# cbg-ethz/metMHN

Hardware: AMD Instinct MI355X
Metric: full-cohort log-lik+grad evals/sec at n=20 events; kronvec HBM GB/s (higher is better)
Workload: dtype f64

## Files before the change

metmhn_amd/csrc/engine.hip:

```cpp
#include <algorithm>
#include <chrono>
#include <cmath>
#include <cstdio>
#include <cstdlib>
#include <cstring>
#include <string>
#include <vector>

#include "../../include/metmhn_amd.h"
#include "host.h"
#include "comm.h"
#include "plan.h"
#include "sampler.h"
#include "rowmix.h"

namespace mmhn {

static thread_local std::string g_err;

struct CListDev {
  DevArr<CItem> items;
  DevArr<int> deps;
};
struct StagedDev {
  DevArr<int> pats, paired, probs;
  DevArr<int2> map, lmap, grc;
  CListDev cl[2];
};
struct BatchDev {
  DevArr<PatRec> pats;
  DevArr<Desc> dJ, dS;
  DevArr<int2> mapJ, mapS, lmapJ, mapX, grcJ, lmapT;
  DevArr<int> sp_list[3][SP_NCLASS], paired, olist, ptoff;
  DevArr<uint32_t> ptiles;
  DevArr<WDesc> wd;
  DevArr<WChain> wchains;
  DevArr<int4> pcl;
  DevArr<double> wrow;
  CListDev clJ[2];
  StagedDev stg[2];
};

struct Config {
  PlanCfg plan;
  bool zero_copy = true;
  bool poison = false;
  bool force_timing = false;
  bool coop_fault = false;
  int coop_wgs = 0;
  bool coop = true;
  long long sim_chunk = 1ll << 26;
  int stream_blocks = 256 * 8;
  bool trace_host = false;
  Config() {
    plan.use_jacobi = env_is("MMHN_SOLVER", "jacobi");
    plan.psolve_min = (int)env_int("MMHN_PSOLVE_MIN", plan.psolve_min);
    plan.wsolve_min = (int)env_int("MMHN_WSOLVE_MIN", env_set("MMHN_PSOLVE_MIN") ? plan.psolve_min : plan.wsolve_min);
    plan.wsolve_mode = (int)env_int("MMHN_WSOLVE", plan.wsolve_mode);
    plan.wsolve_wgs = (int)env_int("MMHN_WSOLVE_WGS", plan.wsolve_wgs);
    plan.prep_split_max = (int)env_int("MMHN_PREP_SPLIT", plan.prep_split_max);
    plan.pcl_per = std::max(1, (int)env_int("MMHN_PCL_PER", plan.pcl_per));
    plan.small_path = env_flag("MMHN_SMALL", plan.small_path);
    zero_copy = env_flag("MMHN_ZEROCOPY", zero_copy);
    poison = env_flag("MMHN_POISON", poison);
    force_timing = env_flag("MMHN_TIME_KERNELS", force_timing);
    coop_fault = env_flag("MMHN_COOP_FAULT", coop_fault);
    coop_wgs = (int)env_int("MMHN_COOP_WGS", coop_wgs);
    coop = env_flag("MMHN_COOP", coop);
    sim_chunk = std::max(1ll, env_int("MMHN_SIM_CHUNK", sim_chunk));
    stream_blocks = (int)env_int("MMHN_STREAM_BLOCKS", stream_blocks);
    trace_host = env_set("MMHN_TRACE_HOST");
  }
};

struct EngineBase {
  virtual ~EngineBase() = default;
  int dtype = 0;
  int device = 0;
  hipStream_t stream = nullptr;
  Config cfg;
};

template <typename T> struct Engine;
template <typename T> void clear_row_groups(Engine<T>& E);
template <typename T> void launch_mix(Engine<T>& E, const Lane& L);

template <typename T>
struct PList {
  const Desc* d; const int2* map; int ntiles; int maxk; long long vec;
  const int2* lmap; const std::vector<int>* lof; const T* tab;
  const CList* cl = nullptr;
  const CListDev* dcl = nullptr;
  int kslot = MMHN_K_OTHER_SOLVE;
};

template <typename... K>
static void raise_lds(size_t bytes, K... kernels) {
  for (const void* k : {reinterpret_cast<const void*>(kernels)...})
    HIPCHECK(hipFuncSetAttribute(k, hipFuncAttributeMaxDynamicSharedMemorySize, (int)bytes));
}

template <typename T>
struct Engine : EngineBase {
  using PList = mmhn::PList<T>;
  int n = 0, N = 0;
  DevArr<Params<T>> d_par;
  Params<T>* h_par = nullptr;
  void* h_par_dev = nullptr;
  DevArr<uint16_t> d_perm;
  DevArr<int> d_lvl;
  std::vector<int8_t> dat;
  long long n_pat = 0;
  int n_cols = 0;
  struct Counts { double em = 0, pat = 0, unknown = 0; } plain, weighted, grouped;
  std::vector<Batch> batches;
  std::vector<BatchDev> dev;
  DevArr<T> pi, lidgJ, qJ, rhsJ, rhsS, pS, lidgS, qS, seedS, GS, dots, bmJ, bmS, tabJ, tabS;
  DevArr<T> piM, qM;
  DevArr<T> zarena;
  struct View { T* p = nullptr; } GJ, DJ, Abuf;
  int pi_owner = -1, qJ_owner = -1;
  DevArr<double> lp, out, sums, abi_sums, redbuf;
  DevArr<double> resp;
  long long n_unknown = 0;
  std::vector<double> row_w;
  std::vector<long long> grp_ptr;
  std::vector<int> grp_rows;
  std::vector<double> grp_w;
  struct GroupsDev {
    DevArr<long long> gptr, mptr;
    DevArr<int> grows, mgrp;
    DevArr<double> gw, lpc, lpg, omega, lambda, rho;
  } gd;
  bool want_rho = false;
  DevArr<JLink<T>> links;
  double* h_abi = nullptr;
  double* h_abi_dev = nullptr;
  Lane main, side[3];
  DevArr<CoopCtl> coop_ctl;
  DevArr<unsigned> coop_flags[2];
  unsigned coop_epoch = 0;
  int coop_slot = 0;
  unsigned* h_abort = nullptr;
  unsigned* h_abort_dev = nullptr;
  bool coop_used = false;
  bool coop_alone = false;
  bool sums_pending = false;
  std::chrono::steady_clock::time_point sums_t0, sums_issued;
  int sums_len = 0;
  int pack_mode = 0;
  double pack_a = 0, pack_b = 0;
  double* pack_dst = nullptr;
  bool packed_in_eval = false;
  double reduce_flag = 0.0, reduce_flag_sum = 0.0;
  bool flag_pending = false;
  ncclComm_t comm = nullptr;
  int comm_rank = 0, comm_size = 1;
  bool time_kernels = true;
  mmhn_counters cnt{};
  std::vector<std::pair<hipEvent_t, hipEvent_t>> ev_pool;
  size_t ev_used = 0;
  std::vector<double> ev_bytes;
  std::vector<int> ev_slot;

  static long long zarena_elems(long long nJ, long long asize, int N) { return up4(3 * nJ * N * N) + up4(3 * nJ * N) + up4(asize); }
  static long long zclear_elems(const Batch& b, int N) { return zarena_elems((long long)b.dJ.size(), b.aclr, N); }

  Engine(int dev_id, int n_mut) : n(n_mut), N(n_mut + 1) {
    device = dev_id;
    cnt.comm_rank = -1;
    REQUIRE(n_mut >= 1 && n_mut < MAXN, "n_mut must be in [1, 31]");
    DevGuard guard(device);
    HIPCHECK(hipStreamCreateWithFlags(&stream, hipStreamNonBlocking));
    main.s = stream;
    main.flags = 0;
    d_par.alloc(NPSET);
    HIPCHECK(hipHostMalloc(reinterpret_cast<void**>(&h_par), NPSET * sizeof(Params<T>), hipHostMallocDefault));
    HIPCHECK(hipHostGetDevicePointer(&h_par_dev, h_par, 0));
    static_assert(sizeof(Params<T>) % sizeof(uint4) == 0, "parameter block: whole 16-byte words");
    sums.alloc(2 * stride());
    size_t free_b = 0, total_b = 0;
    HIPCHECK(hipMemGetInfo(&free_b, &total_b));
    cfg.plan.ws_limit = (size_t)(0.7 * (double)free_b);
    hipDeviceProp_t prop;
    HIPCHECK(hipGetDeviceProperties(&prop, device));
    cfg.plan.n_cu = std::max(1, prop.multiProcessorCount);
    {
      std::vector<uint16_t> perm((size_t)(TB + 1) << TB, 0);
      std::vector<int> lvl((size_t)(TB + 1) * (TB + 2), 0);
      for (int t = 0; t <= TB; ++t) {
        int pos = 0;
        for (int l = 0; l <= t; ++l) {
          lvl[(size_t)t * (TB + 2) + l] = pos;
          for (uint32_t x = 0; x < (1u << t); ++x)
            if (popc(x) == l) perm[((size_t)t << TB) + pos++] = (uint16_t)x;
        }
        lvl[(size_t)t * (TB + 2) + t + 1] = pos;
      }
      d_perm.alloc(perm.size());
      d_lvl.alloc(lvl.size());
      HIPCHECK(hipMemcpy(d_perm.p, perm.data(), perm.size() * sizeof(uint16_t), hipMemcpyHostToDevice));
      HIPCHECK(hipMemcpy(d_lvl.p, lvl.data(), lvl.size() * sizeof(int), hipMemcpyHostToDevice));
    }
    raise_lds(wsolve_lds<T>(), &k_wsolve<T, false>, &k_wsolve<T, true>, &k_wsolve<T, false, WCfg<T>::NXT>, &k_wsolve<T, true, WCfg<T>::NXT>);
    raise_lds(wclass_lds<T>(), &k_wclass<T>);
    raise_lds(160 * 1024, &k_spatient2<T>, &k_spatient<T, 1024, 1>);
    raise_lds(150 * 1024,
              &k_csolve<T, false, false>, &k_csolve<T, true, false>, &k_csolve<T, false, true>, &k_csolve<T, true, true>,
              &k_csolve<T, false, false, 4>, &k_csolve<T, true, false, 4>,
              &k_psolve2<T, false, true>, &k_psolve2<T, true, true>, &k_psolve2<T, false, false>, &k_psolve2<T, true, false>,
              &k_tsolve<T, false, false>, &k_tsolve<T, true, false>, &k_tsolve<T, false, true>, &k_tsolve<T, true, true>,
              &k_kv<T, false, 1, false>, &k_kv<T, true, 1, false>, &k_kv<T, false, 1, true>, &k_kv<T, true, 1, true>,
              &k_sweep<T, false>, &k_sweep<T, true>, &k_diag<T>, &k_diag<T, 1024>,
              &k_prep<T, false>, &k_prep<T, true>, &k_prep<T, false, 1024>, &k_grad_rows<T, 1>, &k_grad_rows<T>,
              &k_pclass<T, false>, &k_pclass<T, true>, &k_class_marg<T>);
    coop_ctl.alloc(1);
    HIPCHECK(hipMemset(coop_ctl.p, 0, sizeof(CoopCtl)));
    HIPCHECK(hipHostMalloc(reinterpret_cast<void**>(&h_abort), 64, hipHostMallocDefault));
    HIPCHECK(hipHostGetDevicePointer(reinterpret_cast<void**>(&h_abort_dev), h_abort, 0));
    *h_abort = 0u;
    for (Lane& l : side) {
      HIPCHECK(hipStreamCreateWithFlags(&l.s, hipStreamNonBlocking));
      HIPCHECK(hipEventCreateWithFlags(&l.ev_fork, hipEventDisableTiming));
      HIPCHECK(hipEventCreateWithFlags(&l.ev_join, hipEventDisableTiming));
    }
    side[2].flags = 1;
  }
  ~Engine() override {
    comm_destroy();
    for (auto& e : ev_pool) { (void)hipEventDestroy(e.first); (void)hipEventDestroy(e.second); }
    for (Lane& l : side) {
      if (l.ev_join) (void)hipEventDestroy(l.ev_join);
      if (l.ev_fork) (void)hipEventDestroy(l.ev_fork);
      if (l.s) (void)hipStreamDestroy(l.s);
    }
    if (h_par) (void)hipHostFree(h_par);
    if (h_abi) (void)hipHostFree(h_abi);
    if (h_abort) (void)hipHostFree(h_abort);
    if (stream) (void)hipStreamDestroy(stream);
    stream = nullptr;
  }
  int stride() const { return 1 + N * N + 2 * N; }

  void build_params(const double* lt, const double* ldp, const double* ldm, bool upload = true) {
    REQUIRE(!sums_pending, "an evaluation begun with mmhn_cohort_sums_begin has not been collected (its parameter upload may still be in flight)");
    std::vector<double> eth((size_t)N * N), enp(N, 1.0), enm(N, 1.0);
    for (int e = 0; e < N * N; ++e) eth[e] = std::exp(lt[e]);
    if (ldp) for (int j = 0; j < N; ++j) enp[j] = std::exp(-ldp[j]);
    if (ldm) for (int j = 0; j < N; ++j) enm[j] = std::exp(-ldm[j]);
// ... 173 lines not shown
    }
    if (!b.lmapT.empty()) {
      const PList LT{db.dJ.p, nullptr, (int)b.lmapT.size(), b.maxkT, 0, db.lmapT.p, &b.lofT, tabJ.p, b.clJ, db.clJ,
                     tr ? MMHN_K_CSOLVE_ADJ : MMHN_K_CSOLVE_FWD};
      solve(L, tr, LT, y, nullptr, nullptr, rhs_mode, nullptr);
    }
  }

  void solve(const Lane& L, bool tr, const PList& P, T* y, const T* lidg, const T* rhs, int rhs_mode, const T* scal) {
    if (P.ntiles == 0) return;
    if (cfg.plan.use_jacobi) {
      zero(L, y, P.vec);
      const double bytes = 4.0 * (double)P.vec * sizeof(T);
      for (int s = 0; s <= P.maxk; ++s)
        launch_sweep(L, tr, P.d, P.map, P.ntiles, P.maxk, y, y, lidg, rhs, rhs_mode, scal, bytes, P.tab);
      return;
    }
    const int nlev = (int)P.lof->size() - 1;
    const size_t lds = sweep_lds(P.maxk);
    const int mk = std::max(P.maxk, 1);
    const double per_tile = (double)((rhs_mode == 0 ? 2 : 1) + (lidg ? 1 : 0)) * (double)(1 << std::min(P.maxk, TB)) * sizeof(T);
    if (cfg.coop && P.cl && nlev > 1) {
      const CList& cl = P.cl[tr ? 1 : 0];
      const CListDev& dcl = P.dcl[tr ? 1 : 0];
      const int nitems = (int)cl.items.size();
      REQUIRE(nitems == P.ntiles, "cooperative solve: work list and tile list differ");
      REQUIRE(L.flags >= 0, "cooperative solve: issued on a lane without a flag set");
      DevArr<unsigned>& flags = coop_flags[L.flags];
      if (flags.n < (size_t)nitems) {
        HIPCHECK(hipStreamSynchronize(L.s));
        flags.alloc((size_t)nitems + 1024);
        HIPCHECK(hipMemsetAsync(flags.p, 0, flags.n * sizeof(unsigned), L.s));
      }
      if (++coop_epoch == 0u) {
        HIPCHECK(hipDeviceSynchronize());
        for (auto& f : coop_flags) if (f.p) HIPCHECK(hipMemset(f.p, 0, f.n * sizeof(unsigned)));
        coop_epoch = 1u;
      }
      coop_slot = (coop_slot + 1) & 3;
      const int slot = L.flags * 4 + coop_slot;
      coop_used = true;
      timed(L, P.kslot, per_tile * nitems, [&]() {
        const dim3 g((unsigned)std::min(nitems, cfg.coop_wgs > 0 ? cfg.coop_wgs : cfg.plan.n_cu)), bk(TSB);
#define CS_ARGS g, bk, lds, L.s, P.d, dcl.items.p, dcl.deps.p, nitems, flags.p, coop_epoch, coop_ctl.p, slot, h_abort_dev, cfg.coop_fault ? 1 : 0, \
                y, lidg, rhs, rhs_mode, scal, d_perm.p, mk, P.tab, links.p, qS.p
        with_flags([&](auto tr_) {
          if (lidg) hipLaunchKernelGGL((k_csolve<T, tr_(), true>), CS_ARGS);
          else if (coop_alone) hipLaunchKernelGGL((k_csolve<T, tr_(), false, 4>), CS_ARGS);
          else hipLaunchKernelGGL((k_csolve<T, tr_(), false>), CS_ARGS);
        }, tr);
#undef CS_ARGS
      });
      return;
    }
    for (int s = 0; s < nlev; ++s) {
      const int lev = tr ? nlev - 1 - s : s;
      const int beg = (*P.lof)[lev], cntl = (*P.lof)[lev + 1] - beg;
      if (cntl == 0) continue;
      timed(L, P.kslot, per_tile * cntl, [&]() {
        with_flags([&](auto tr_, auto jac) {
          hipLaunchKernelGGL((k_tsolve<T, tr_(), jac()>), dim3(cntl), dim3(TSB), lds, L.s, P.d, P.lmap + beg, d_par.p, y, lidg, rhs, rhs_mode, scal,
                             d_perm.p, d_lvl.p, mk, P.tab, links.p, qS.p);
        }, tr, lidg != nullptr);
      });
    }
  }
  void check_abort() {
    if (!coop_used) return;
    coop_used = false;
    if (*h_abort == 0u) return;
    *h_abort = 0u;
    (void)hipMemset(coop_ctl.p, 0, sizeof(CoopCtl));
    throw Fail{"cooperative tile solve: a wait for another workgroup's tile timed out (results discarded)"};
  }

  void upload(const Batch& b, BatchDev& d) {
    auto up = [](auto& to, const auto& host) {
      if (host.empty()) return;
      to.alloc(host.size());
      HIPCHECK(hipMemcpy(to.p, host.data(), host.size() * sizeof(host[0]), hipMemcpyHostToDevice));
    };
    auto up_clist = [&](CListDev& to, const CList& cl) { up(to.items, cl.items); up(to.deps, cl.deps); };
    up(d.pats, b.pats); up(d.dJ, b.dJ); up(d.dS, b.dS);
    up(d.mapJ, b.mapJ); up(d.mapS, b.mapS); up(d.lmapJ, b.lmapJ); up(d.mapX, b.mapX); up(d.grcJ, b.grcJ);
    up(d.wd, b.wd); up(d.wchains, b.wchains); up(d.olist, b.olist); up(d.ptoff, b.ptoff); up(d.ptiles, b.ptiles);
    up(d.lmapT, b.lmapT); up_clist(d.clJ[0], b.clJ[0]); up_clist(d.clJ[1], b.clJ[1]);
    up(d.pcl, b.pcl); up(d.paired, b.paired);
    for (int w = 0; w < 3; ++w) for (int c = 0; c < SP_NCLASS; ++c) up(d.sp_list[w][c], b.sp_list[w][c]);
    for (int w = 0; w < 2; ++w) {
      const Staged& g = b.stg[w];
      StagedDev& dg = d.stg[w];
      up(dg.pats, g.pats); up(dg.paired, g.paired); up(dg.probs, g.probs);
      up(dg.map, g.map); up(dg.lmap, g.lmap); up(dg.grc, g.grc);
      up_clist(dg.cl[0], g.cl[0]); up_clist(dg.cl[1], g.cl[1]);
    }
  }
  void set_cohort(const int8_t* d_, long long np, int nc) {
    REQUIRE(nc == 2 * n + 3, "dat must have 2*n_mut+3 columns");
    REQUIRE(np >= 0, "negative patient count");
    REQUIRE(!sums_pending, "mmhn_set_cohort: an evaluation begun with mmhn_cohort_sums_begin has not been collected");
    dat.assign(d_, d_ + np * nc);
    n_pat = np;
    n_cols = nc;
    batches.clear();
    dev.clear();
    row_w.clear();
    clear_row_groups(*this);
    n_unknown = 0;
    plain = Counts{0, (double)np, 0};
    try {
      batches = plan_cohort<T>(cfg.plan, dat.data(), np, nc, n, plain.em);
      for (long long r = 0; r < np; ++r) n_unknown += dat[(size_t)r * nc + nc - 1] == 4;
      plain.unknown = (double)n_unknown;
      place_cohort();
    } catch (...) {
      dat.clear(); batches.clear(); dev.clear();
      n_pat = 0; n_unknown = 0;
      plain = Counts{};
      throw;
    }
  }
  bool mixing() const { return !grp_ptr.empty(); }
  const Counts& counts() const { return mixing() ? grouped : row_w.empty() ? plain : weighted; }
  void row_weight_sums(double* out3) const { out3[0] = counts().em; out3[1] = counts().pat; out3[2] = counts().unknown; }
  void place_cohort() {
    dev.resize(batches.size());
    long long mvJ = 0, mvS = 0, mtJ = 0, mtS = 0, mvM = 0;
    size_t mZ = 0, mnJ = 0, mnS = 0, mp = 0;
    for (const Batch& b : batches) {
      upload(b, dev[b.id]);
      mvJ = std::max(mvJ, b.vecJ); mvS = std::max(mvS, b.vecS);
      mZ = std::max<size_t>(mZ, (size_t)zarena_elems((long long)b.dJ.size(), b.asize, N));
      mtJ = std::max(mtJ, b.tabJ); mtS = std::max(mtS, b.tabS);
      if (b.wpath && !b.wdirect) mvM = std::max(mvM, b.vecJ);
      mnJ = std::max(mnJ, b.dJ.size()); mnS = std::max(mnS, b.dS.size()); mp = std::max(mp, b.pats.size());
    }
    pi.alloc(mvJ); qJ.alloc(mvJ);
    piM.alloc(mvM); qM.alloc(mvM);
    if (cfg.plan.use_jacobi) { lidgJ.alloc(mvJ); rhsJ.alloc(mvJ); }
    links.alloc(std::max<size_t>(mnJ, 1));
    tabJ.alloc(mtJ); tabS.alloc(mtS);
    pi_owner = qJ_owner = -1;
    rhsS.alloc(mvS); pS.alloc(mvS); lidgS.alloc(mvS); qS.alloc(mvS);
    seedS.alloc(mnS);
    GS.alloc(mnS * N * N); zarena.alloc(mZ);
    dots.alloc(2 * mp); bmJ.alloc(mnJ * 64); bmS.alloc(mnS * 64);
    resp.alloc((size_t)std::max<long long>(n_pat, 1));
    {
      const std::vector<double> nans(resp.n, std::nan(""));
      HIPCHECK(hipMemcpy(resp.p, nans.data(), resp.n * sizeof(double), hipMemcpyHostToDevice));
    }
    lp.alloc(mp); out.alloc(mp * stride()); redbuf.alloc(((mp + red_per((int)mp) - 1) / red_per((int)mp)) * 2 * (size_t)stride());
  }

  void small_classes(const Batch& b, int which, bool grad) {
    const BatchDev& db = dev[b.id];
    const int n0 = (int)b.sp_list[which][0].size(), n1 = (int)b.sp_list[which][1].size(), n2 = (int)b.sp_list[which][2].size();
    const int np0 = which ? (int)b.sp_list[2][0].size() : 0, np1 = which ? (int)b.sp_list[2][1].size() : 0;
    const int mk0 = spatient_class_maxk(0), mk1 = which ? b.mk1p : spatient_class_maxk(1), mk2 = spatient_class_maxk(2);
    const bool on_side = which == 0 ? (n0 + n1 + n2 > 0) : n2 > 0;
    Lane& sd = side[which];
    if (on_side) sd.begin(main);
    else sd.reset();
#define SP_TAIL db.pats.p, db.dS.p, d_par.p, d_perm.p, d_lvl.p, db.dJ.p, db.wd.p, pi.p, links.p, pS.p, qS.p, GS.p, bmS.p, dots.p, lp.p, resp.p
    if (n2) {
      const size_t lds = (spatient_lds<T>(N, mk2) + 15) / 16 * 16;
      hipLaunchKernelGGL((k_spatient<T, 1024, 1>), dim3(n2), dim3(1024), lds, sd.s, db.sp_list[which][2].p, n2, SP_TAIL, mk2, N, grad ? 1 : 0);
      HIPCHECK(hipGetLastError());
    }
    if (n0 + n1 + np0 + np1) {
      const size_t s0 = (spatient_lds<T>(N, mk0) + 15) / 16 * 16, s1 = (spatient_lds<T>(N, mk1) + 15) / 16 * 16;
      const size_t lds = std::max(s0 * SP_PPB0, n1 + np1 ? s1 * (np1 ? 2 : 1) : 0) + 64;
      const int nblk = (n0 + SP_PPB0 - 1) / SP_PPB0 + n1 + (np0 + SP_PPB0 / 2 - 1) / (SP_PPB0 / 2) + np1;
      hipLaunchKernelGGL((k_spatient2<T>), dim3(nblk), dim3(256), lds, which == 0 ? sd.s : main.s,
                         db.sp_list[which][0].p, n0, mk0, db.sp_list[which][1].p, n1, mk1,
                         db.sp_list[2][0].p, np0, db.sp_list[2][1].p, np1, SP_TAIL, N, grad ? 1 : 0);
      HIPCHECK(hipGetLastError());
    }
#undef SP_TAIL
    if (on_side) sd.end();
  }

  bool eval_head(const double* lt, const double* ldp, const double* ldm, bool grad) {
    const int st = stride();
    bool head_done = false;
    if (cfg.zero_copy && !batches.empty()) {
      build_params(lt, ldp, ldm, false);
      const Batch& b0 = batches.front();
      long long nz = grad && !b0.dJ.empty() ? zclear_elems(b0, N) * (long long)sizeof(T) / 16 : 0;
      const bool fill_here = nz <= (32ll << 20) / 16;
      if (!fill_here) nz = 0;
      const int nw = (int)(NPSET * sizeof(Params<T>) / sizeof(uint4));
      const long long need = std::max<long long>(std::max<long long>(nw, 2 * st), nz);
      const int nblk = (int)std::min<long long>((need + 255) / 256, 4096);
      hipLaunchKernelGGL(k_begin_eval, dim3(nblk), dim3(256), 0, main.s, static_cast<const uint4*>(h_par_dev),
                         reinterpret_cast<uint4*>(d_par.p), nw, sums.p, 2 * st, reinterpret_cast<uint4*>(zarena.p), nz);
      HIPCHECK(hipGetLastError());
      head_done = fill_here;
    } else {
      build_params(lt, ldp, ldm);
      HIPCHECK(hipMemsetAsync(sums.p, 0, 2 * st * sizeof(double), main.s));
    }
    if (mixing() && cfg.poison) HIPCHECK(hipMemsetAsync(gd.lpc.p, 0xFF, (size_t)n_pat * sizeof(double), main.s));
    return head_done;
  }
  void batch_prepare(const Batch& b, bool grad, bool cleared) {
    const int nJ = (int)b.dJ.size();
    coop_alone = b.stg[0].empty();
    time_kernels = cfg.force_timing || b.vecJ + b.vecS >= (1ll << 26);
    GJ.p = zarena.p;
    DJ.p = GJ.p + up4(3ll * nJ * N * N);
    Abuf.p = DJ.p + up4(3ll * nJ * N);
    if (grad && nJ && !cleared) zero(main, zarena.p, zclear_elems(b, N));
    if (grad && nJ && cfg.poison) poison_fill(main, Abuf.p + b.aclr, b.asize - b.aclr);
  }
  void clear_dead_tiles(const Batch& b, bool grad) {
    if (cfg.plan.use_jacobi || b.dJ.empty()) return;
    if (pi_owner != b.id) { zero(main, pi.p + b.offT, b.vecJ - b.offT); pi_owner = b.id; }
    if (grad && qJ_owner != b.id) { zero(main, qJ.p + b.offT, b.vecJ - b.offT); qJ_owner = b.id; }
    if (cfg.poison && b.offT > 0) {
      HIPCHECK(hipMemsetAsync(pi.p, 0xFF, (size_t)b.offT * sizeof(T), main.s));
      if (grad) HIPCHECK(hipMemsetAsync(qJ.p, 0xFF, (size_t)b.offT * sizeof(T), main.s));
    }
  }
  PList joint_list(const Batch& b) const {
    const BatchDev& db = dev[b.id];
    return PList{db.dJ.p, db.mapJ.p, (int)b.mapJ.size(), b.maxkJ, b.vecJ, db.lmapJ.p, &b.lofJ, tabJ.p};
  }
  void joint_forward(const Batch& b) {
    const BatchDev& db = dev[b.id];
    if (cfg.plan.use_jacobi) {
      launch_diag(main, db.dJ.p, db.mapJ.p, (int)b.mapJ.size(), nullptr, lidgJ.p, nullptr, KD_LIDG);
      solve(main, false, joint_list(b), pi.p, lidgJ.p, nullptr, 2, nullptr);
    } else {
      psolve(main, false, b, pi.p, 2);
    }
  }
  PList staged_list(const Batch& b, int w) const {
    const Staged& g = b.stg[w];
    const StagedDev& dg = dev[b.id].stg[w];
    return PList{dev[b.id].dS.p, dg.map.p, (int)g.map.size(), g.maxk, b.vecS, dg.lmap.p, &g.lof, tabS.p, g.cl, dg.cl};
  }
  void staged_fwd(const Lane& L, const Batch& b, int w, bool grad) {
    const BatchDev& db = dev[b.id];
    const Staged& g = b.stg[w];
    const StagedDev& dg = db.stg[w];
    if (g.empty()) return;
    const int nG = (int)g.pats.size(), tG = (int)g.map.size();
    hipLaunchKernelGGL((k_staged_init<T>), dim3(nG), dim3(BLOCK), 0, L.s, db.pats.p, db.dS.p, rhsS.p, GS.p, bmS.p, N, grad ? 1 : 0, dg.pats.p);
    HIPCHECK(hipGetLastError());
    prep(L, db.dS.p, (int)g.probs.size(), tabS.p, false, 0, dg.probs.p);
    if (!g.paired.empty()) {
      hipLaunchKernelGGL((k_gather_marg<T>), dim3((unsigned)g.paired.size(), 2, g.maxk > 10 ? 8 : 1), dim3(BLOCK), 0, L.s,
                         db.pats.p, db.dJ.p, db.dS.p, d_par.p, pi.p, rhsS.p, links.p, dg.paired.p, db.wd.p);
      HIPCHECK(hipGetLastError());
    }
    launch_diag(L, db.dS.p, dg.map.p, tG, nullptr, lidgS.p, nullptr, KD_LIDG);
    solve(L, false, staged_list(b, w), pS.p, lidgS.p, rhsS.p, 0, nullptr);
    hipLaunchKernelGGL((k_seeds<T>), dim3((nG + 255) / 256), dim3(256), 0, L.s, db.pats.p, nG, db.dS.p,
                       d_par.p, pS.p, seedS.p, lp.p, resp.p, N, dg.pats.p);
    HIPCHECK(hipGetLastError());
  }
  void staged_adj(const Lane& L, const Batch& b, int w) {
    const BatchDev& db = dev[b.id];
    const Staged& g = b.stg[w];
    const StagedDev& dg = db.stg[w];
    if (g.empty()) return;
    solve(L, true, staged_list(b, w), qS.p, lidgS.p, nullptr, 1, seedS.p);
    launch_grad_rows(L, db.dS.p, (int)g.probs.size(), g.maxk, nullptr, pS.p, qS.p, GS.p, GK_S, dg.grc);
    if (g.kind2) {
      hipLaunchKernelGGL((k_bit_marg<T>), dim3((unsigned)g.map.size()), dim3(BLOCK), 0, L.s, db.dS.p, dg.map.p, d_par.p, pS.p, qS.p, bmS.p);
      HIPCHECK(hipGetLastError());
    }
  }
  void joint_adjoint(const Batch& b) {
    const BatchDev& db = dev[b.id];
    if (cfg.plan.use_jacobi) zero(main, rhsJ.p, b.vecJ);
    for (int part = 0; part < 2 && !b.stg[1].paired.empty(); ++part) {
      if (b.stg[1].paired.size() >= 256)
        hipLaunchKernelGGL((k_scatter_marg<T, 1024>), dim3((unsigned)b.stg[1].paired.size()), dim3(1024), 0, main.s, db.pats.p, db.dJ.p,
                           db.dS.p, d_par.p, qS.p, rhsS.p, cfg.plan.use_jacobi ? rhsJ.p : nullptr, dots.p, part, db.stg[1].paired.p);
      else
        hipLaunchKernelGGL((k_scatter_marg<T>), dim3((unsigned)b.stg[1].paired.size()), dim3(BLOCK), 0, main.s, db.pats.p, db.dJ.p,
                           db.dS.p, d_par.p, qS.p, rhsS.p, cfg.plan.use_jacobi ? rhsJ.p : nullptr, dots.p, part, db.stg[1].paired.p);
      HIPCHECK(hipGetLastError());
    }
    if (cfg.plan.use_jacobi) solve(main, true, joint_list(b), qJ.p, lidgJ.p, rhsJ.p, 0, nullptr);
    else psolve(main, true, b, qJ.p, 3);
  }
  void joint_gradient(const Batch& b) {
    const BatchDev& db = dev[b.id];
    const int nJ = (int)b.dJ.size();
    if (!cfg.plan.use_jacobi) {
      const double mbytes = (double)b.vecJ * sizeof(T);
      timed(main, MMHN_K_PCLASS, mbytes, [&]() {
        if (b.wdirect) {
          const int nW = (int)b.wd.size();
// ... 975 lines not shown
```

metmhn_amd/csrc/gradrows.h:

```cpp
#pragma once
#include "common.h"

namespace mmhn {

enum { GK_P = 0, GK_M = 1, GK_E = 2, GK_S = 3 };

template <typename T>
__device__ __forceinline__ T wave_sum(T v) {
  for (int o = 32; o > 0; o >>= 1) v += __shfl_xor(v, o);
  return v;
}

template <int CTRL, int ROWMASK>
__device__ __forceinline__ double dpp_add(double v) {
  const int lo = __builtin_amdgcn_update_dpp(0, __double2loint(v), CTRL, ROWMASK, 0xF, false);
  const int hi = __builtin_amdgcn_update_dpp(0, __double2hiint(v), CTRL, ROWMASK, 0xF, false);
  return v + __hiloint2double(hi, lo);
}
template <int CTRL, int ROWMASK>
__device__ __forceinline__ float dpp_add(float v) {
  return v + __int_as_float(__builtin_amdgcn_update_dpp(0, __float_as_int(v), CTRL, ROWMASK, 0xF, false));
}
__device__ __forceinline__ double lane63(double v) {
  return __hiloint2double(__builtin_amdgcn_readlane(__double2hiint(v), 63), __builtin_amdgcn_readlane(__double2loint(v), 63));
// ... 78 lines not shown
  const bool drow = i == N;
  if (i > N || (drow && (kind == GK_S || DJ == nullptr))) return;
  T* row = drow ? DJ + ((long long)kind * nprob + prob) * N : G + ((long long)prob * N + i) * N;
  T* rb = rowbuf + w * 32;
  if (lane < 32) rb[lane] = 0;
  const T* fvec = drow ? (kind == GK_M ? P.dm : P.dp) : P.th[i < N ? i : 0];

  bool rowvalid = true;
  T base = drow ? (kind == GK_P ? -P.dp[n] : kind == GK_M ? -P.dm[n] : T(-1)) : (kind == GK_M ? P.baseM[i] : P.baseP[i]);
  if ((kind == GK_P || kind == GK_M) && ((!drow && i >= n) || d.seedbit < 0)) rowvalid = false;
  if (kind == GK_E && d.mode != JOINT) rowvalid = false;
  int slot = -1;
  if (drow) slot = -1;
  else if (kind == GK_E && i == n) slot = kc;
  else for (int l = 0; l < kc; ++l) if (lev[l] == i) slot = l;

  if (rowvalid) {
    const int klo = kc < 6 ? kc : 6;
    const int kin = kc < GR_CHUNK ? kc : GR_CHUNK;
    const int nhi = kin - klo;
    const T fl = lane < kc ? fvec[lev[lane < kc ? lane : 0]] : T(1);
#pragma unroll
    for (int part = 0; part < 3; ++part) {
      T v = 1;
#pragma unroll
      for (int l = 0; l < 6; ++l) {
        const int ll = part * 6 + l;
        const T f = lane_bcast(fl, ll);
        if (ll < kc && ((lane >> l) & 1)) v *= f;
      }
      Tlo[w * 192 + part * 64 + lane] = v;
    }
    constexpr int NHI = GR_CHUNK - 6;
    T ha[NHI];
#pragma unroll
    for (int l = 0; l < NHI; ++l) ha[l] = 0;
    const T* Ab = nullptr;
    if (kind != GK_S) {
      long long o = d.aoff;
      if (kind != GK_P) o += class_block_size(__popc(d.maskP));
      if (kind == GK_E) o += class_block_size(__popc(d.maskM));
      Ab = A + o;
    }
    const long long nS = 1ll << kc;
    const long long Sbeg = (long long)chunk << GR_CHUNK;
    const long long Send = nS < Sbeg + (1ll << GR_CHUNK) ? nS : Sbeg + (1ll << GR_CHUNK);
    T tot = 0;
    constexpr int GU = 4;
    for (long long S00 = Sbeg; S00 < Send; S00 += 64 * GU) {
      T a0[GU], a1[GU];
      bool live[GU];
#pragma unroll
      for (int u = 0; u < GU; ++u) {
        const long long S = S00 + 64 * u + lane;
        const uint32_t s = (uint32_t)S;
        const bool blocked = slot >= 0 && slot < kc && ((s >> slot) & 1u);
        live[u] = S < nS && !blocked;
        a0[u] = 0; a1[u] = 0;
        if (live[u]) {
          if (kind == GK_S) {
            const T pv = p[d.off + s];
            a0[u] = -pv * q[d.off + s];
            if (slot >= 0) a1[u] = pv * q[d.off + (s | (1u << slot))];
          } else {
            a0[u] = Ab[S];
            if (slot >= 0) a1[u] = Ab[((long long)(slot + 1) << kc) + S];
          }
        }
      }
#pragma unroll
      for (int u = 0; u < GU; ++u) {
        const long long S0 = S00 + 64 * u;
        if (S0 >= nS) break;
        const uint32_t s = (uint32_t)(S0 + lane);
        T urate = base;
        urate *= Tlo[w * 192 + 64 + ((S0 >> 6) & 63)] * Tlo[w * 192 + 128 + ((S0 >> 12) & 63)];
        for (int l = 18; l < kc; ++l) if ((S0 >> l) & 1) urate *= fvec[lev[l]];
        const T f = live[u] ? urate * Tlo[w * 192 + (s & 63u)] * (a0[u] + a1[u]) : T(0);
        tot += f;
#pragma unroll
        for (int l = 0; l < NHI; ++l) if (l < nhi && ((S0 >> (6 + l)) & 1)) ha[l] += f;
      }
    }
    const T total = wave_sum(tot);
    if (lane == 0) {
      if (drow) { if (kind != GK_E) rb[n] = total; }
      else { rb[i] = total; if (kind == GK_M) rb[n] = total; }
    }
    for (int l = 0; l < klo; ++l) {
      const T m = wave_sum(((lane >> l) & 1) ? tot : T(0));
      if (lane == 0 && lev[l] != i) rb[lev[l]] = m;
    }
#pragma unroll
    for (int l = 0; l < NHI; ++l) {
      if (l < nhi) {
        const T m = wave_sum(ha[l]);
        if (lane == 0 && lev[6 + l] != i) rb[lev[6 + l]] = m;
      }
    }
    if (lane == 0)
      for (int l = kin; l < kc; ++l)
        if (((Sbeg >> l) & 1) && lev[l] != i) rb[lev[l]] = total;
  }
  if (lane < N && rb[lane] != T(0)) atomicAdd(&row[lane], rb[lane]);
}

template <typename T>
__global__ __launch_bounds__(BLOCK) void k_bit_marg(const Desc* __restrict__ descs,
                                                    const int2* __restrict__ map,
                                                    const Params<T>* __restrict__ par,
                                                    const T* __restrict__ p,
                                                    const T* __restrict__ q, T* out) {
  __shared__ T part[WAVES][2][16];
  const Desc& d = descs[map[blockIdx.x].x];
  const uint32_t H = (uint32_t)map[blockIdx.x].y;
  const int k = d.k, n = d.N - 1;
  const int t = k < TB ? k : TB;
  const uint32_t nelem = 1u << t;
  const Params<T>& P = par[d.pset];
  const bool joint = d.mode == JOINT;
  const int tid = threadIdx.x, w = tid >> 6, lane = tid & 63;
  constexpr int NJ = (1 << TB) / BLOCK;
  T tot[2] = {0, 0};
  T mj[2][4] = {{0, 0, 0, 0}, {0, 0, 0, 0}};
#pragma unroll
  for (int j = 0; j < NJ; ++j) {
    const uint32_t xl = (uint32_t)j * BLOCK + tid;
    if (xl < nelem) {
      const uint32_t x = (H << t) | xl;
      T a = 1, b = 1;
      for (int bb = 0; bb < k; ++bb)
        if ((x >> bb) & 1u) {
          if (joint ? d.cls[bb] == CP : bb != d.seedbit) a *= P.dp[d.ev[bb]];
          if (joint ? d.cls[bb] == CM : bb != d.seedbit) b *= P.dm[d.ev[bb]];
        }
      const bool sbit = d.seedbit >= 0 && ((x >> d.seedbit) & 1u);
      T wA, wB;
      if (joint) { wA = sbit ? a * P.dp[n] : a; wB = sbit ? b * P.dm[n] : T(0); }
      else { wA = sbit ? T(0) : a; wB = sbit ? b * P.dm[n] : T(0); }
      const T pq = p[d.off + x] * q[d.off + x];
      const T vA = pq * wA, vB = pq * wB;
      tot[0] += vA; tot[1] += vB;
#pragma unroll
      for (int l = 0; l < 4; ++l) if ((j >> l) & 1) { mj[0][l] += vA; mj[1][l] += vB; }
    }
  }
#pragma unroll
  for (int ww = 0; ww < 2; ++ww) {
    const T s = wave_sum(tot[ww]);
    if (lane == 0) part[w][ww][12] = s;
#pragma unroll
    for (int l = 0; l < 6; ++l) {
      const T m = wave_sum(((lane >> l) & 1) ? tot[ww] : T(0));
      if (lane == 0) part[w][ww][l] = m;
    }
    if (lane == 0) { part[w][ww][6] = (w & 1) ? s : T(0); part[w][ww][7] = (w & 2) ? s : T(0); }
#pragma unroll
    for (int l = 0; l < 4; ++l) {
      const T m = wave_sum(mj[ww][l]);
      if (lane == 0) part[w][ww][8 + l] = m;
    }
  }
  __syncthreads();
  T* o = out + (long long)map[blockIdx.x].x * 64;
  if (tid < 2 * 32) {
    const int ww = tid >> 5, b = tid & 31;
    if (b < k) {
      T m = 0;
      if (b < t) { for (int v = 0; v < WAVES; ++v) m += part[v][ww][b]; }
      else if ((H >> (b - t)) & 1u) { for (int v = 0; v < WAVES; ++v) m += part[v][ww][12]; }
      if (m != T(0)) atomicAdd(&o[ww * 32 + b], m);
    }
  }
}

}
```

metmhn_amd/csrc/plan.h:

```cpp
#pragma once
#include <algorithm>
#include <cmath>
#include <cstdint>
#include <string>
#include <vector>

#include "host.h"
#include "kernels.h"
#include "tsolve.h"
#include "small.h"
#include "wsolve.h"
#include "wclass.h"

namespace mmhn {

struct PlanCfg {
  size_t ws_limit = 0;
  int n_cu = 256;
  bool use_jacobi = false;
  int wsolve_mode = 1;
  int wsolve_min = 128;
  int psolve_min = 384;
  int wsolve_wgs = 0;
  int prep_split_max = 2048;
  int pcl_per = 16;
  bool small_path = true;
};

struct CList {
  std::vector<CItem> items;
  std::vector<int> deps;
  int maxk = 0;
  int nlevels = 0;
  void clear() { items.clear(); deps.clear(); maxk = 0; nlevels = 0; }
};
enum Route : uint8_t { RT_W = 0, RT_P = 1, RT_T = 2 };

struct Staged {
  std::vector<int> pats, paired, probs;
  std::vector<int2> map, lmap;
  std::vector<int> lof;
  std::vector<int2> grc;
  CList cl[2];
  int maxk = 0;
  bool kind2 = false;
  bool empty() const { return pats.empty(); }
};

struct Batch {
  std::vector<PatRec> pats;
  std::vector<Desc> dJ, dS;
  std::vector<int2> mapJ, mapS;
  long long vecJ = 0, vecS = 0, asize = 0, tabJ = 0, tabS = 0;
  long long aclr = 0;
  int id = 0;
  int maxkJ = 0;
  int maxkcJ = 0;
  std::vector<int2> lmapJ;
  std::vector<int> lofJ;
  std::vector<int2> mapX;
  std::vector<int2> grcJ;
  std::vector<int> sp_list[3][SP_NCLASS];
  bool has_small = false;
  int mk1p = 9;
  Staged stg[2];
  std::vector<int> paired;
  std::vector<uint8_t> route;
  std::vector<int> olist;
  bool wpath = false;
  bool wdirect = false;
  std::vector<WDesc> wd;
  int wnx = -1;
  std::vector<WChain> wchains;
  long long offT = 0;
  CList clJ[2];
  std::vector<int2> lmapT;
  std::vector<int> lofT;
  int maxkT = 0, maxkP = 0;
  int max_dl = 0;
  std::vector<int> ptoff;
  std::vector<uint32_t> ptiles;
  std::vector<int4> pcl;
};

inline long long up4(long long v) { return (v + 3) / 4 * 4; }

static bool dead_tile(const Desc& d, uint32_t H) {
  if (d.mode != JOINT || d.seedbit < TB) return false;
  const uint32_t xhi = H << TB, hmask = ~((1u << TB) - 1u);
  if (xhi & (1u << d.seedbit)) return false;
  if (xhi & d.lone & hmask) return true;
  const uint32_t pp = d.pairP & hmask & ~(1u << 31);
  const uint32_t pm = (pp << 1);
  if (((xhi & pp) << 1) != (xhi & pm)) return true;
  return false;
}

static void build_levels(const std::vector<int2>& map, const std::vector<Desc>* descs, bool prune,
                         std::vector<int2>& lmap, std::vector<int>& lof) {
  int maxl = 0;
  std::vector<int2> keep;
  keep.reserve(map.size());
  for (const int2& m : map) {
    if (prune && descs && dead_tile((*descs)[m.x], (uint32_t)m.y)) continue;
    keep.push_back(m);
    maxl = std::max(maxl, popc((uint32_t)m.y));
  }
  lof.assign(maxl + 2, 0);
  for (const int2& m : keep) lof[popc((uint32_t)m.y) + 1]++;
  for (int l = 0; l <= maxl; ++l) lof[l + 1] += lof[l];
  lmap.resize(keep.size());
  std::vector<int> cur(lof.begin(), lof.end() - 1);
  for (const int2& m : keep) lmap[cur[popc((uint32_t)m.y)]++] = m;
}

static inline long long a_size(const Desc& d) {
  const int kP = popc(d.maskP), kM = popc(d.maskM), kE = popc(d.pairP);
  return ((long long)(kP + 1) << kP) + ((long long)(kM + 1) << kM) + ((long long)(kE + 2) << kE);
}

static void add_tiles(std::vector<int2>& map, int prob, int k) {
  const int tiles = k > TB ? 1 << (k - TB) : 1;
  for (int t = 0; t < tiles; ++t) map.push_back(make_int2(prob, t));
}

static void tile_deps(const Desc& d, uint32_t H, bool tr, std::vector<uint32_t>& out) {
  out.clear();
  const int k = d.k, t = k < TB ? k : TB;
  const bool joint = d.mode == JOINT;
  for (int b = (t > 0 ? t - 1 : 0); b < k; ++b) {
    const bool is_pair = joint && ((d.pairP >> b) & 1u);
    for (int kind = 0; kind < 2; ++kind) {
      if (kind == 1 && !is_pair) continue;
      const uint32_t mv = kind == 0 ? (1u << b) : (3u << b);
      const uint32_t mh = mv >> t;
      if (mh == 0) continue;
      if (tr ? (H & mh) != 0 : (H & mh) != mh) continue;
      const uint32_t Hn = H ^ mh;
      if (std::find(out.begin(), out.end(), Hn) == out.end()) out.push_back(Hn);
    }
  }
}

static void build_clist(const std::vector<int2>& map, const std::vector<Desc>& descs, bool prune, bool tr, CList& cl) {
  cl.clear();
  struct Ent { int prob; uint32_t H; int key; int k; };
  std::vector<Ent> ents;
  ents.reserve(map.size());
  std::vector<int> maxlev(descs.size(), 0);
  for (const int2& m : map) {
    if (prune && dead_tile(descs[m.x], (uint32_t)m.y)) continue;
    maxlev[m.x] = std::max(maxlev[m.x], popc((uint32_t)m.y));
    ents.push_back(Ent{m.x, (uint32_t)m.y, 0, descs[m.x].k});
  }
  if (ents.empty()) return;
  for (Ent& e : ents) {
    const int lev = popc(e.H);
    e.key = tr ? -lev : lev - maxlev[e.prob];
    cl.maxk = std::max(cl.maxk, e.k);
    cl.nlevels = std::max(cl.nlevels, maxlev[e.prob] + 1);
  }
  std::stable_sort(ents.begin(), ents.end(), [](const Ent& a, const Ent& b) { return a.key != b.key ? a.key < b.key : a.k > b.k; });
  std::vector<long long> toff(descs.size() + 1, 0);
  std::vector<char> used(descs.size(), 0);
  for (const Ent& e : ents) used[e.prob] = 1;
  for (size_t p = 0; p < descs.size(); ++p) toff[p + 1] = toff[p] + (used[p] ? (descs[p].k > TB ? 1ll << (descs[p].k - TB) : 1) : 0);
  std::vector<int> pos((size_t)toff.back(), -1);
  for (size_t i = 0; i < ents.size(); ++i) pos[(size_t)(toff[ents[i].prob] + ents[i].H)] = (int)i;
  cl.items.resize(ents.size());
  std::vector<uint32_t> nb;
  for (size_t i = 0; i < ents.size(); ++i) {
    const Ent& e = ents[i];
    tile_deps(descs[e.prob], e.H, tr, nb);
    CItem it{e.prob, e.H, (int)cl.deps.size(), 0};
    for (uint32_t Hn : nb) {
      const int j = pos[(size_t)(toff[e.prob] + Hn)];
      if (j < 0) continue;
      if (j >= (int)i) throw Fail{"cooperative solve: the work list is not a topological order"};
      cl.deps.push_back(j);
      ++it.ndep;
    }
    if (it.ndep > 63) throw Fail{"cooperative solve: more than 63 dependencies of one tile"};
    cl.items[i] = it;
  }
  if (cl.deps.empty()) cl.deps.push_back(0);
}

static std::vector<int2> grad_chunks(const std::vector<Desc>& ds, int kind) {
  std::vector<int2> out;
  for (size_t i = 0; i < ds.size(); ++i) {
    const Desc& d = ds[i];
    const int kc = kind == GK_P ? popc(d.maskP) : kind == GK_M ? popc(d.maskM) : kind == GK_E ? popc(d.pairP) : d.k;
    const int nch = 1 << std::max(0, kc - GR_CHUNK);
    for (int c = 0; c < nch; ++c) out.push_back(int2{(int)i, c});
  }
  return out;
}

struct CutTargets {
  double soft = 0;
  long long pats = 0;
};
template <typename T>
static CutTargets batch_targets(const PlanCfg& c, const int8_t* dat, long long np, int nc, int n) {
  CutTargets t;
  double total = 0;
  long long npJ = 0;
  for (long long r = 0; r < np; ++r) {
    const int8_t* row = dat + r * nc;
    int kp = 0, km = 0, ke = 0;
    for (int j = 0; j < n; ++j) { kp += row[2 * j] != 0; km += row[2 * j + 1] != 0; ke += row[2 * j] && row[2 * j + 1]; }
    const int type = row[nc - 1];
    double el = 0;
    if (type == 3) {
      ++npJ;
      el = (c.use_jacobi || c.wsolve_mode == 2 ? 4.0 : 2.0) * std::ldexp(1.0, kp + km + 1) + 4.0 * (std::ldexp(1.0, km + 1) + std::ldexp(1.0, kp + 1)) +
           (kp + 1) * std::ldexp(1.0, kp) + (km + 1) * std::ldexp(1.0, km) + (ke + 2) * std::ldexp(1.0, ke);
    } else if (type == 4) {
      el = 4.0 * (std::ldexp(1.0, kp) + std::ldexp(1.0, kp + 1));
    } else {
      el = 4.0 * std::ldexp(1.0, (type == 2 ? km : kp) + 1);
    }
    total += el * sizeof(T);
  }
  const double nb = std::ceil(total / (double)std::max<size_t>(c.ws_limit, 1));
  t.soft = nb > 1 ? total / nb * 1.02 : 0;
  if (nb > 1 && npJ > 0) {
    const double per_batch = (double)c.ws_limit / (total / (double)npJ);
    if (per_batch >= (double)c.n_cu) {
      t.pats = (long long)(per_batch / c.n_cu) * c.n_cu;
      const long long nbt = (npJ + t.pats - 1) / t.pats, rem = npJ - (nbt - 1) * t.pats;
      if (nbt > 1 && rem < std::max(c.psolve_min, c.wsolve_min)) t.pats = (npJ + nbt - 1) / nbt;
    }
  }
  return t;
}

struct RowProblems {
  PatRec pr{};
  Desc dj{}, ds[2]{};
  bool hasJ = false, has[2] = {false, false};
};
static RowProblems decode_row(const int8_t* row, long long r, int n, int nc) {
  const int type = row[nc - 1];
  const int order = row[nc - 2];
  const std::string at = " (row " + std::to_string(r) + ")";
  REQUIRE(type >= 0 && type <= 4, "dat: type column must be 0..4" + at);
  for (int c = 0; c < 2 * n + 1; ++c) REQUIRE(row[c] == 0 || row[c] == 1, "dat: event columns must be 0/1");
  if (type == 4) {
    for (int j = 0; j < n; ++j) REQUIRE(row[2 * j + 1] == 0, "dat: rows of unknown status (type 4) must have no MT event" + at);
    REQUIRE(row[2 * n] == 0, "dat: rows of unknown status (type 4) must have seeding = 0" + at);
  }
  RowProblems p;
  PatRec& pr = p.pr;
  pr.kind = type; pr.order = (order == 0 || order == 1) ? order : 2; pr.j = -1; pr.s[0] = pr.s[1] = -1;
  pr.row = (int)r;
  int npt = 0, nmt = 0;
  for (int j = 0; j < n; ++j) { npt += row[2 * j]; nmt += row[2 * j + 1]; }
  const int kmax = type == 4 ? npt + 1 : type == 3 ? npt + nmt + 1 : type == 2 ? nmt + 1 : npt + row[2 * n];
  const bool unseeded_pair = type == 3 && row[2 * n] != 1;
  REQUIRE(unseeded_pair || kmax <= MAXK, type == 4 ? "too many active events for one patient" + at : std::string("too many active events for one patient"));
  std::vector<int8_t> st(2 * n + 2);
  if (type == 4) {
    pr.kind = 5;
    for (int j = 0; j < n; ++j) st[j] = row[2 * j];
    st[n] = 0;
    if (npt > 0) { p.ds[0] = make_single(st.data(), n, PS_PRIM, OBS_ONE); p.has[0] = true; }
    st[n] = 1;
    p.ds[1] = make_single(st.data(), n, PS_PRIM, OBS_ONE);
    p.has[1] = true;
  } else if (type == 0 || type == 1) {
    for (int j = 0; j <= n; ++j) st[j] = row[2 * j];
    int np_ = 0;
    for (int j = 0; j <= n; ++j) np_ += st[j];
    if (type == 0 && np_ == 0) pr.kind = 4;
    else { p.ds[0] = make_single(st.data(), n, PS_PRIM, OBS_ONE); p.has[0] = true; }
  } else if (type == 2) {
    for (int j = 0; j < n; ++j) st[j] = row[2 * j + 1];
    st[n] = 1;
// ... 217 lines not shown
static void assign_small_classes(const PlanCfg& c, int N, Batch& b) {
  for (int w = 0; w < 3; ++w) for (int cl = 0; cl < SP_NCLASS; ++cl) b.sp_list[w][cl].clear();
  for (int w = 0; w < 2; ++w) { Staged& g = b.stg[w]; g.pats.clear(); g.paired.clear(); g.probs.clear(); g.kind2 = false; }
  bool class_fits[SP_NCLASS];
  for (int cl = 0; cl < SP_NCLASS; ++cl)
    class_fits[cl] = (spatient_lds<T>(N, spatient_class_maxk(cl)) + 15) / 16 * 16 * (size_t)(cl == 0 ? SP_PPB0 : cl == 1 ? 2 : 1) + 64 <= (size_t)160 * 1024;
  const bool all_staged = !c.small_path || c.use_jacobi;
  for (size_t pi_ = 0; pi_ < b.pats.size(); ++pi_) {
    const PatRec& pr = b.pats[pi_];
    int ks = -1;
    for (int part = 0; part < 2; ++part) if (pr.s[part] >= 0) ks = std::max(ks, b.dS[pr.s[part]].k);
    if (ks < 0) continue;
    int cl = 0;
    while (cl < SP_NCLASS - 1 && ks > spatient_class_maxk(cl)) ++cl;
    if (all_staged || ks > TB || !class_fits[cl]) {
      Staged& g = b.stg[all_staged || pr.j >= 0 ? 1 : 0];
      g.pats.push_back((int)pi_);
      if (pr.j >= 0) g.paired.push_back((int)pi_);
      for (int part = 0; part < 2; ++part) if (pr.s[part] >= 0) g.probs.push_back(pr.s[part]);
      if (pr.kind == 2) g.kind2 = true;
      continue;
    }
    const bool side_by_side = pr.j >= 0 && pr.s[0] >= 0 && pr.s[1] >= 0 && cl < 2;
    b.sp_list[side_by_side ? 2 : pr.j >= 0 ? 1 : 0][cl].push_back((int)pi_);
  }
  b.mk1p = spatient_class_maxk(1);
  if (!b.sp_list[1][2].empty() && b.sp_list[1][2].size() <= 16) {
    int mk = 0;
    for (int pi_ : b.sp_list[1][2])
      for (int part = 0; part < 2; ++part) if (b.pats[pi_].s[part] >= 0) mk = std::max(mk, b.dS[b.pats[pi_].s[part]].k);
    if (mk <= 10 && (spatient_lds<T>(N, mk) + 15) / 16 * 16 * 2 + 64 <= (size_t)160 * 1024) {
      for (int pi_ : b.sp_list[1][2]) b.sp_list[b.pats[pi_].s[0] >= 0 && b.pats[pi_].s[1] >= 0 ? 2 : 1][1].push_back(pi_);
      b.sp_list[1][2].clear();
      b.mk1p = mk;
    }
  }
  auto ksize = [&](int pi_) {
    const PatRec& pr = b.pats[pi_];
    int ks = 0;
    for (int part = 0; part < 2; ++part) if (pr.s[part] >= 0) ks = std::max(ks, 64 * b.dS[pr.s[part]].k + (pr.s[0] >= 0 && pr.s[1] >= 0 ? 32 : 0) + pr.kind);
    return ks;
  };
  b.has_small = false;
  for (int w = 0; w < 3; ++w)
    for (int cl = 0; cl < SP_NCLASS; ++cl) {
      std::stable_sort(b.sp_list[w][cl].begin(), b.sp_list[w][cl].end(), [&](int x, int y) { return ksize(x) > ksize(y); });
      if (!b.sp_list[w][cl].empty()) b.has_small = true;
    }
}

static void build_staged_groups(const PlanCfg& c, Batch& b) {
  const std::vector<int2> chunks = grad_chunks(b.dS, GK_S);
  for (int w = 0; w < 2; ++w) {
    Staged& g = b.stg[w];
    std::vector<char> isg(b.dS.size(), 0);
    for (int sp : g.probs) isg[sp] = 1;
    g.map.clear(); g.maxk = 0;
    for (const int2& m : b.mapS) if (isg[m.x]) { g.map.push_back(m); g.maxk = std::max(g.maxk, b.dS[m.x].k); }
    build_levels(g.map, nullptr, false, g.lmap, g.lof);
    g.cl[0].clear(); g.cl[1].clear();
    if (!c.use_jacobi && g.lof.size() > 2) { build_clist(g.map, b.dS, false, false, g.cl[0]); build_clist(g.map, b.dS, false, true, g.cl[1]); }
    g.grc.clear();
    for (const int2& e : chunks) if (isg[e.x]) g.grc.push_back(e);
  }
}

static void layout_class_arrays(const PlanCfg& c, Batch& b) {
  const int nJ = (int)b.dJ.size();
  b.wdirect = b.wpath && c.wsolve_mode != 2;
  long long ao = 0;
  for (int pj = 0; pj < nJ; ++pj) if (!(b.wdirect && b.route[pj] == RT_W)) { b.dJ[pj].aoff = ao; ao += a_size(b.dJ[pj]); }
  b.aclr = up4(ao);
  ao = b.aclr;
  for (int pj = 0; pj < nJ; ++pj) if (b.wdirect && b.route[pj] == RT_W) { b.dJ[pj].aoff = ao; ao += a_size(b.dJ[pj]); }
  b.asize = ao;
  for (Desc& dj : b.dJ) dj.wl = -1;
  if (b.wdirect) for (size_t i = 0; i < b.wd.size(); ++i) b.dJ[b.wd[i].prob].wl = (int)i;
}

static void build_grad_chunks(Batch& b) {
  b.grcJ.clear();
  for (int kd = 0; kd < 3; ++kd)
    for (const int2& e : grad_chunks(b.dJ, kd)) b.grcJ.push_back(int2{e.x, e.y | (kd << 24)});
}

template <typename T>
static std::vector<Batch> plan_cohort(const PlanCfg& c, const int8_t* dat, long long np, int nc, int n, double& n_em) {
  const int N = n + 1;
  std::vector<Batch> batches = split_into_batches<T>(c, dat, np, nc, n, n_em);
  for (Batch& b : batches) {
    route_joint_problems<T>(c, b);
    layout_joint_vectors(b);
    build_window_chains<T>(c, b);
    build_tile_route(c, b);
    build_psolve_tiles(b);
    build_pclass_items(c, b);
    build_index_lists(c, b);
    assign_small_classes<T>(c, N, b);
    build_staged_groups(c, b);
    layout_class_arrays(c, b);
    build_grad_chunks(b);
  }
  return batches;
}

}
```

Measured before the change: 22.73.

## Skip zeroing gradient rows for single-chunk problems; fuse wave bit-sums

Gradient row buffers (GJ/DJ) are no longer zero-filled wholesale each evaluation. Problems whose lattice fits in one chunk now store their row directly instead of using atomicAdd. Only multi-chunk problems are cleared, by a small per-problem kernel, and the zero arena is shrunk to the A buffer. Separately, the per-bit wave reductions in the gradient row kernel are replaced with a combined wave_bit_sums and DPP reductions, which cuts cross-lane shuffle work. This trades memset bandwidth for an extra kernel launch and relies on every GJ/DJ entry being written by exactly one chunk.

```diff
diff --git a/metmhn_amd/csrc/engine.hip b/metmhn_amd/csrc/engine.hip
--- a/metmhn_amd/csrc/engine.hip
+++ b/metmhn_amd/csrc/engine.hip
@@ -30,7 +30,7 @@
 struct BatchDev {
   DevArr<PatRec> pats;
   DevArr<Desc> dJ, dS;
-  DevArr<int2> mapJ, mapS, lmapJ, mapX, grcJ, lmapT;
+  DevArr<int2> mapJ, mapS, lmapJ, mapX, grcJ, gclrJ, lmapT;
   DevArr<int> sp_list[3][SP_NCLASS], paired, olist, ptoff;
   DevArr<uint32_t> ptiles;
   DevArr<WDesc> wd;
@@ -164,7 +164,7 @@
   std::vector<int> ev_slot;
 
   static long long zarena_elems(long long nJ, long long asize, int N) { return up4(3 * nJ * N * N) + up4(3 * nJ * N) + up4(asize); }
-  static long long zclear_elems(const Batch& b, int N) { return zarena_elems((long long)b.dJ.size(), b.aclr, N); }
+  static long long zclear_elems(const Batch& b) { return up4(b.aclr); }
 
   Engine(int dev_id, int n_mut) : n(n_mut), N(n_mut + 1) {
     device = dev_id;
@@ -504,7 +504,8 @@
     };
     auto up_clist = [&](CListDev& to, const CList& cl) { up(to.items, cl.items); up(to.deps, cl.deps); };
     up(d.pats, b.pats); up(d.dJ, b.dJ); up(d.dS, b.dS);
-    up(d.mapJ, b.mapJ); up(d.mapS, b.mapS); up(d.lmapJ, b.lmapJ); up(d.mapX, b.mapX); up(d.grcJ, b.grcJ);
+    up(d.mapJ, b.mapJ); up(d.mapS, b.mapS); up(d.lmapJ, b.lmapJ); up(d.mapX, b.mapX);
+    up(d.grcJ, b.grcJ); up(d.gclrJ, b.gclrJ);
     up(d.wd, b.wd); up(d.wchains, b.wchains); up(d.olist, b.olist); up(d.ptoff, b.ptoff); up(d.ptiles, b.ptiles);
     up(d.lmapT, b.lmapT); up_clist(d.clJ[0], b.clJ[0]); up_clist(d.clJ[1], b.clJ[1]);
     up(d.pcl, b.pcl); up(d.paired, b.paired);
@@ -609,7 +610,7 @@
     if (cfg.zero_copy && !batches.empty()) {
       build_params(lt, ldp, ldm, false);
       const Batch& b0 = batches.front();
-      long long nz = grad && !b0.dJ.empty() ? zclear_elems(b0, N) * (long long)sizeof(T) / 16 : 0;
+      long long nz = grad && !b0.dJ.empty() ? zclear_elems(b0) * (long long)sizeof(T) / 16 : 0;
       const bool fill_here = nz <= (32ll << 20) / 16;
       if (!fill_here) nz = 0;
       const int nw = (int)(NPSET * sizeof(Params<T>) / sizeof(uint4));
@@ -630,11 +631,16 @@
     const int nJ = (int)b.dJ.size();
     coop_alone = b.stg[0].empty();
     time_kernels = cfg.force_timing || b.vecJ + b.vecS >= (1ll << 26);
-    GJ.p = zarena.p;
+    Abuf.p = zarena.p;
+    GJ.p = Abuf.p + up4(b.asize);
     DJ.p = GJ.p + up4(3ll * nJ * N * N);
-    Abuf.p = DJ.p + up4(3ll * nJ * N);
-    if (grad && nJ && !cleared) zero(main, zarena.p, zclear_elems(b, N));
-    if (grad && nJ && cfg.poison) poison_fill(main, Abuf.p + b.aclr, b.asize - b.aclr);
+    if (grad && nJ && !cleared) zero(main, zarena.p, zclear_elems(b));
+    if (grad && nJ && cfg.poison) poison_fill(main, Abuf.p + b.aclr, zarena_elems(nJ, b.asize, N) - b.aclr);
+    if (grad && !b.gclrJ.empty()) {
+      hipLaunchKernelGGL((k_grad_clear<T>), dim3((unsigned)b.gclrJ.size()), dim3(BLOCK), 0, main.s, dev[b.id].gclrJ.p, GJ.p, DJ.p, N, nJ,
+                         (long long)nJ * N * N);
+      HIPCHECK(hipGetLastError());
+    }
   }
   void clear_dead_tiles(const Batch& b, bool grad) {
     if (cfg.plan.use_jacobi || b.dJ.empty()) return;
diff --git a/metmhn_amd/csrc/gradrows.h b/metmhn_amd/csrc/gradrows.h
--- a/metmhn_amd/csrc/gradrows.h
+++ b/metmhn_amd/csrc/gradrows.h
@@ -184,19 +184,19 @@
         for (int l = 0; l < NHI; ++l) if (l < nhi && ((S0 >> (6 + l)) & 1)) ha[l] += f;
       }
     }
-    const T total = wave_sum(tot);
+    T total, M[6] = {0, 0, 0, 0, 0, 0};
+    wave_bit_sums(tot, lane, klo, total, M);
     if (lane == 0) {
       if (drow) { if (kind != GK_E) rb[n] = total; }
       else { rb[i] = total; if (kind == GK_M) rb[n] = total; }
     }
-    for (int l = 0; l < klo; ++l) {
-      const T m = wave_sum(((lane >> l) & 1) ? tot : T(0));
-      if (lane == 0 && lev[l] != i) rb[lev[l]] = m;
-    }
+#pragma unroll
+    for (int l = 0; l < 6; ++l)
+      if (l < klo && lane == 0 && lev[l] != i) rb[lev[l]] = M[l];
 #pragma unroll
     for (int l = 0; l < NHI; ++l) {
       if (l < nhi) {
-        const T m = wave_sum(ha[l]);
+        const T m = wave_sum_dpp(ha[l]);
         if (lane == 0 && lev[6 + l] != i) rb[lev[6 + l]] = m;
       }
     }
@@ -204,7 +204,17 @@
       for (int l = kin; l < kc; ++l)
         if (((Sbeg >> l) & 1) && lev[l] != i) rb[lev[l]] = total;
   }
-  if (lane < N && rb[lane] != T(0)) atomicAdd(&row[lane], rb[lane]);
+  if (kc <= GR_CHUNK) { if (lane < N) row[lane] = rb[lane]; }
+  else if (lane < N && rb[lane] != T(0)) atomicAdd(&row[lane], rb[lane]);
+}
+
+template <typename T>
+__global__ __launch_bounds__(BLOCK) void k_grad_clear(const int2* __restrict__ items, T* __restrict__ G, T* __restrict__ DJ, int N,
+                                                      int nprob, long long gstride) {
+  const int prob = items[blockIdx.x].x, kind = items[blockIdx.x].y;
+  T* g = G + (long long)kind * gstride + (long long)prob * N * N;
+  for (int e = threadIdx.x; e < N * N; e += BLOCK) g[e] = T(0);
+  if ((int)threadIdx.x < N) DJ[((long long)kind * nprob + prob) * N + threadIdx.x] = T(0);
 }
 
 template <typename T>
diff --git a/metmhn_amd/csrc/plan.h b/metmhn_amd/csrc/plan.h
--- a/metmhn_amd/csrc/plan.h
+++ b/metmhn_amd/csrc/plan.h
@@ -60,6 +60,7 @@
   std::vector<int> lofJ;
   std::vector<int2> mapX;
   std::vector<int2> grcJ;
+  std::vector<int2> gclrJ;
   std::vector<int> sp_list[3][SP_NCLASS];
   bool has_small = false;
   int mk1p = 9;
@@ -195,6 +196,10 @@
     for (int c = 0; c < nch; ++c) out.push_back(int2{(int)i, c});
   }
   return out;
+}
+
+static inline int grad_lattice_bits(const Desc& d, int kind) {
+  return kind == GK_P ? popc(d.maskP) : kind == GK_M ? popc(d.maskM) : kind == GK_E ? popc(d.pairP) : d.k;
 }
 
 struct CutTargets {
@@ -578,6 +583,10 @@
   b.grcJ.clear();
   for (int kd = 0; kd < 3; ++kd)
     for (const int2& e : grad_chunks(b.dJ, kd)) b.grcJ.push_back(int2{e.x, e.y | (kd << 24)});
+  b.gclrJ.clear();
+  for (int kd = 0; kd < 3; ++kd)
+    for (size_t p = 0; p < b.dJ.size(); ++p)
+      if (grad_lattice_bits(b.dJ[p], kd) > GR_CHUNK) b.gclrJ.push_back(int2{(int)p, kd});
 }
 
 template <typename T>
```

After: 22.71. About the same (-0.1%).
